# millecker/hadoop-1.0.3-gpu

Hardware: AMD Instinct MI355X
Metric: K-Means job makespan + map-tasks/sec (whole node) at 1/2/4/8 MI355X (higher is better)
Workload: dtype fp32

## Files before the change

hbmr/models/kmeans.py:

```python
from __future__ import annotations

import base64
import logging
import math
import os
import threading
import time

import numpy as np
import torch

from ..gpu.splitjob import SplitJob, SplitSpec
from ..mapred import counters as C

log = logging.getLogger("hbmr.kmeans")

K_KEY = "hbmr.kmeans.k"
D_KEY = "hbmr.kmeans.dims"
INPUT_KEY = "hbmr.kmeans.input"
SPLIT_PTS_KEY = "hbmr.split.points"
CIN_KEY = "hbmr.kmeans.centroids.in"
COUT_KEY = "hbmr.kmeans.centroids.out"
INIT_KEY = "hbmr.kmeans.centroids.init"
NCENTERS_KEY = "hbmr.kmeans.synthetic.centers"
RETURN_KEY = "hbmr.kmeans.return.centroids"
CDIR_KEY = "hbmr.kmeans.centroids.dir"
EXACT_KEY = "hbmr.kmeans.exact"
EXACT_MFMA_KEY = "hbmr.kmeans.exact.mfma"
COMBINER_KEY = "hbmr.kmeans.combiner"
BOUNDS_KEY = "hbmr.kmeans.exact.bounds"

_M32 = 0xFFFFFFFF


def _mix32(x: torch.Tensor) -> torch.Tensor:
    x = x & _M32
    x = ((x ^ (x >> 16)) * 0x45D9F3B) & _M32
    x = ((x ^ (x >> 16)) * 0x45D9F3B) & _M32
    return x ^ (x >> 16)


def _uniform(c: torch.Tensor) -> torch.Tensor:
    return (_mix32(c).to(torch.float64) + 0.5) * (1.0 / 4294967296.0)


def _gauss(c1: torch.Tensor, c2: torch.Tensor) -> torch.Tensor:
    u1 = _uniform(c1)
    u2 = _uniform(c2)
    return torch.sqrt(-2.0 * torch.log(u1)) * torch.cos(2.0 * math.pi * u2)


def synthetic_points(seed: int, start: int, n: int, d: int, centers: int, device,
                     chunk: int = 1 << 18) -> torch.Tensor:
# ... 236 lines not shown
            t = _EXACT_SKIPPED[key] = torch.zeros(1, dtype=torch.int64, device=device)
        return t


class KMeansSplitJob(SplitJob):
    collective_reduce = True
    needs_reduce = True

    def configure(self, conf):
        self.conf = conf
        self.k = conf.get_int(K_KEY, 64)
        self.d = conf.get_int(D_KEY, 128)
        self.input = conf.get(INPUT_KEY, "synthetic:100000:1")
        self.split_points = conf.get_int(SPLIT_PTS_KEY, 500_000)
        self.cin = conf.get(CIN_KEY)
        self.cout = conf.get(COUT_KEY)
        self.centers = conf.get_int(NCENTERS_KEY, self.k)
        self.fx_shift = conf.get_int("hbmr.kmeans.fx.shift", 24)
        self.cdir = conf.get(CDIR_KEY)
        self.exact = conf.get_boolean(EXACT_KEY, False)
        self.exact_dtype = torch.bfloat16 if (conf.get(EXACT_MFMA_KEY) or "f16").lower() in (
            "bf16", "bfloat16") else torch.float16
        self.bounds = conf.get_boolean(BOUNDS_KEY, True)
        self.combiner = (conf.get(COMBINER_KEY) or "delta").lower()
        if self.combiner not in ("delta", "sorted"):
            raise ValueError(f"{COMBINER_KEY} must be delta or sorted, not {self.combiner!r}")
        init = conf.get(INIT_KEY)
        if init and self.cin and STORE.host_centroids(self.cin) is None:
            STORE.put_host(self.cin, decode_centroids(init))
        if self.cin and self.cdir and STORE.host_centroids(self.cin) is None:
            path = _centroid_file(self.cdir, self.cin)
            if os.path.exists(path):
                STORE.put_host(self.cin, torch.from_numpy(np.load(path)))

    _split_memo: dict = {}

    def get_splits(self, conf, trackers):
        if self.input.startswith("synthetic:"):
            mk = (self.input, self.split_points, self.d, self.centers, tuple(trackers),
                  self.exact)
            got = KMeansSplitJob._split_memo.get(mk)
            if got is not None:
                return got
            if len(KMeansSplitJob._split_memo) > 16:
                KMeansSplitJob._split_memo.clear()
            out = KMeansSplitJob._split_memo[mk] = self._synthetic_splits(trackers)
# ... 215 lines not shown
        B = len(datas)
        sums = torch.empty(B, self.k, img.dp, dtype=torch.int64, device=ctx.device)
        counts = torch.empty(B, self.k, dtype=torch.int64, device=ctx.device)
        order = have + new + plain
        pos = {i: j for j, i in enumerate(order)}
        H = len(have)
        installed = []
        grown = None
        if have:
            ns = [datas[i].shape[0] for i in have]
            total = sum(ns)
            lab = scratch.get("labcat")
            if lab is None or lab.numel() < total:
                lab = scratch["labcat"] = torch.empty(total, dtype=torch.int32, device=ctx.device)
            need = km.delta_workspace_bytes(total, H, self.k)
            if scratch.get("dws") is None or scratch["dws"].numel() < need:
                scratch["dws"] = torch.empty(need, dtype=torch.uint8, device=ctx.device)
            hb = [bases[i] for i in have]
            bounded = self.bounds and self.combiner == "delta" and km.bounds_supported(img)
            if bounded:
                nogap = [b for b in hb if b.gap is None]
                km.assign_exact_batch([datas[i] for i in have], img, stats, lab, scratch,
                                      stream=ctx.stream, bounds=hb,
                                      skipped=_exact_skipped(self.cin, ctx.device))
                grown = {id(b): b.gap.numel() * b.gap.element_size() for b in nogap}
            else:
                km.assign_exact_batch([datas[i] for i in have], img, stats, lab, scratch,
                                      stream=ctx.stream)
            km.delta_combine([datas[i].x32 for i in have], lab, self.k, sums[:H], counts[:H],
                             scratch["dws"], hb, fx_shift=img.fx_shift, stream=ctx.stream,
                             keep_bounds=bounded)
            for i, b in zip(have, hb):
                b.S0, b.N0 = sums[pos[i]], counts[pos[i]]
                installed.append((keys[i], b))
        for i in new + plain:
            d = datas[i]
            s, c = sums[pos[i]], counts[pos[i]]
            s.zero_()
            c.zero_()
            lab = km.assign_exact(d, img, stats, scratch, stream=ctx.stream)
            need = km.workspace_bytes(d.shape[0], img.k)
            if scratch.get("ws") is None or scratch["ws"].numel() < need:
                scratch["ws"] = torch.empty(max(need, 1 << 20), dtype=torch.uint8,
                                            device=ctx.device)
            km.accumulate(d.x32, lab, img.k, s, c, fx_shift=img.fx_shift, stream=ctx.stream,
                          workspace=scratch["ws"])
            if keys[i] is not None and i in new:
# ... 386 lines not shown
```

hbmr/ops/_lib.py:

```python
from __future__ import annotations

import ctypes
import os
import threading
from pathlib import Path

import torch

_LIB_PATH = Path(__file__).resolve().parent.parent / "lib" / "libhbmr.so"
_lock = threading.Lock()
_lib = None

c_void_p = ctypes.c_void_p
c_long = ctypes.c_long
c_int = ctypes.c_int
c_uint = ctypes.c_uint
c_uint64 = ctypes.c_uint64
c_double_p = ctypes.POINTER(ctypes.c_double)

_SIGS = {
    "hbmr_kmeans_assign_bf16": (c_int, [c_void_p, c_long, c_int, c_void_p, c_void_p, c_int,
                                        c_void_p, c_void_p, c_void_p]),
    "hbmr_kmeans_accum_bf16": (c_int, [c_void_p, c_long, c_int, c_void_p, c_int, c_void_p,
                                       c_void_p, c_int, c_void_p, c_long, c_int, c_void_p]),
# ... 27 lines not shown
    "hbmr_kmeans_get_exact_kernel": (c_int, []),
    "hbmr_kmeans_refine_f32": (c_int, [c_void_p, c_long, c_int, c_int, c_void_p, c_void_p,
                                       c_void_p, c_void_p, c_int, c_int, c_void_p, c_void_p,
                                       c_void_p, c_void_p, c_void_p, c_void_p, c_int, c_void_p,
                                       c_void_p, c_void_p, c_void_p, c_void_p, c_int,
                                       c_void_p]),
    "hbmr_kmeans_refine_batch_bytes": (c_long, [c_int, c_void_p]),
    "hbmr_kmeans_assign_top3_grouped": (c_int, [c_int, c_void_p, c_void_p, c_int, c_int,
                                                c_void_p, c_void_p, c_int, c_void_p, c_void_p,
                                                c_void_p, c_void_p, c_void_p]),
    "hbmr_kmeans_refine_batch_q1g": (c_int, [c_int, c_void_p, c_int, c_int, c_int, c_void_p,
                                             c_void_p, c_void_p, c_void_p, c_void_p, c_void_p,
                                             c_void_p, c_void_p, c_void_p, c_void_p, c_void_p,
                                             c_void_p, c_long, c_void_p, c_void_p]),
    "hbmr_kmeans_refine_batch_q1": (c_int, [c_int, c_void_p, c_int, c_int, c_int, c_int,
                                            c_void_p, c_void_p, c_void_p, c_void_p, c_void_p,
                                            c_void_p, c_void_p, c_void_p, c_void_p, c_void_p,
                                            c_void_p, c_void_p, c_void_p, c_long, c_int,
                                            c_void_p, c_void_p]),
    "hbmr_kmeans_refine_batch_finish": (c_int, [c_int, c_void_p, c_void_p, c_void_p, c_int,
                                                c_int, c_void_p, c_int, c_int, c_void_p,
                                                c_void_p, c_void_p, c_void_p, c_int, c_void_p,
                                                c_int, c_void_p, c_long, c_void_p]),
    "hbmr_kmeans_accum_workspace_bytes": (c_long, [c_long, c_int]),
    "hbmr_kmeans_batch_workspace_bytes": (c_long, [c_long, c_int, c_int]),
    "hbmr_kmeans_map_batch": (c_int, [c_int, c_void_p, c_void_p, c_int, c_void_p, c_void_p, c_int,
                                      c_int, c_void_p, c_void_p, c_long, c_void_p, c_void_p,
                                      c_int, c_int, c_void_p]),
    "hbmr_kmeans_delta_workspace_bytes": (c_long, [c_long, c_int, c_int]),
    "hbmr_kmeans_delta_combine": (c_int, [c_int, c_void_p, c_void_p, c_int, c_int, c_int,
                                          c_void_p, c_void_p, c_long, c_void_p, c_void_p, c_int,
                                          c_void_p, c_void_p, c_void_p, c_void_p]),
    "hbmr_kmeans_map_batch_delta": (c_int, [c_int, c_void_p, c_void_p, c_int, c_void_p, c_void_p,
                                            c_int, c_int, c_void_p, c_void_p, c_long, c_void_p,
                                            c_void_p, c_int, c_void_p, c_void_p, c_void_p,
                                            c_void_p]),
    "hbmr_kmeans_update": (c_int, [c_void_p, c_void_p, c_int, c_int, c_int, c_int, c_int,
                                   c_void_p, c_void_p, c_void_p, c_void_p, c_void_p]),
    "hbmr_kmeans_padded_k": (c_int, [c_int]),
    "hbmr_kmeans_map_cpu_f32": (c_int, [c_void_p, c_long, c_int, c_void_p, c_int, c_void_p,
                                        c_void_p, c_void_p, c_double_p, c_int, c_int]),
    "hbmr_kmeans_map_cpu_f32_ex": (c_int, [c_void_p, c_long, c_int, c_void_p, c_int, c_void_p,
                                           c_void_p, c_void_p, c_double_p, c_int, c_int, c_int,
                                           c_void_p]),
    "hbmr_kmeans_padded_dim": (c_int, [c_int]),
    "hbmr_f32_to_bf16_pad": (c_int, [c_void_p, c_long, c_int, c_int, c_void_p, c_void_p]),
# ... 148 lines not shown
```

hbmr/ops/kmeans.py:

```python
from __future__ import annotations

import ctypes
import os
import threading

import torch

from . import _lib
from ..utils.trace import TRACE

SUPPORTED_DP = (64, 128, 256)


def _nullctx():
    import contextlib
    return contextlib.nullcontext()
FX_SHIFT = 24
NBR_L = 256


def padded_dim(d: int) -> int:
    for dp in SUPPORTED_DP:
        if d <= dp:
            return dp
# ... 302 lines not shown
        self.splits, self.img, self.stats, self.stream = splits, img, stats, stream
        self.dt = splits[0].xb.dtype
        self.ns, self.ws = _refine_ws([sp.shape[0] for sp in splits], splits[0].x32.device,
                                      scratch)
        with torch.cuda.stream(stream) if stream is not None else _nullctx():
            self.norms = img.norms(self.dt)
            self.nbr = img.neighbors()
            self.pd = img.pair_dist()
        self.labels = [None] * len(splits)
        self.lib = _lib.load()
        self.st = _lib.stream_handle(stream)

    def q1(self, i, labels_ptr, cand, scores, margin):
        sp, img = self.splits[i], self.img
        cn, cmax, ce, cemax = self.norms
        self.labels[i] = labels_ptr
        rc = self.lib.hbmr_kmeans_refine_batch_q1(
            len(self.splits), self.ns, i, img.d, img.k, img.k_pad, _ptr(sp.xnorm),
            _ptr(sp.xbn2), _ptr(sp.xerr), _ptr(cn), _ptr(cmax), _ptr(ce), _ptr(cemax),
            labels_ptr, _ptr(cand), _ptr(scores), _ptr(margin), _ptr(self.stats),
            _ptr(self.ws), self.ws.numel(), int(i == 0), _ptr(self.pd), self.st)
        _lib.check(rc, "hbmr_kmeans_refine_batch_q1")

    def finish(self):
        B = len(self.splits)
        img = self.img
        _, cmax, _, cemax = self.norms
        ni, nd, L = self.nbr
        xs = (ctypes.c_void_p * B)(*[sp.x32.data_ptr() for sp in self.splits])
        ls = (ctypes.c_void_p * B)(*[(lp.value if isinstance(lp, ctypes.c_void_p) else lp)
                                     for lp in self.labels])
        rc = self.lib.hbmr_kmeans_refine_batch_finish(
            B, self.ns, xs, ls, img.d, self.splits[0].x32.shape[1], _ptr(img.cen), img.k,
            img.k_pad, _ptr(cmax), _ptr(cemax), _ptr(ni), _ptr(nd), L, _ptr(self.stats),
            self.stats.numel(), _ptr(self.ws), self.ws.numel(), self.st)
        _lib.check(rc, "hbmr_kmeans_refine_batch_finish")


def refine_f32(split: ExactSplit, img: CentroidImage, labels, cand, scores, margin,
               stats: torch.Tensor, stream=None, scratch: dict | None = None) -> None:
    n = split.shape[0]
    if stats.dtype != torch.int64 or stats.numel() < 3:
        raise ValueError("stats must be int64 [3]")
    if labels.numel() != n or cand.numel() != 2 * n or margin.numel() != 2 * n:
        raise ValueError("labels [n], cand/margin [2n] from assign_top3 expected")
    if REFINE_VERSION >= 3:
        rb = _RefineBatch([split], img, stats, scratch, stream)
        rb.q1(0, labels.data_ptr(), cand, scores, margin)
        rb.finish()
        return
    with torch.cuda.stream(stream) if stream is not None else _nullctx():
        cn, cmax, ce, cemax = img.norms(split.xb.dtype)
        ni, nd, L = img.neighbors()
    rc = _lib.load().hbmr_kmeans_refine_f32(
        _ptr(split.x32), n, img.d, split.x32.shape[1], _ptr(split.xnorm), _ptr(split.xbn2),
        _ptr(split.xerr), _ptr(img.cen), img.k, img.k_pad, _ptr(cn), _ptr(cmax), _ptr(ce),
        _ptr(cemax), _ptr(ni), _ptr(nd), L,
        _ptr(labels), _ptr(cand), _ptr(scores), _ptr(margin), _ptr(stats), stats.numel(),
        _lib.stream_handle(stream))
# ... 6 lines not shown
    n = split.shape[0]
    dev = split.xb.device
    scratch = {} if scratch is None else scratch
    key = ("exact", n)
    bufs = scratch.get(key)
    if bufs is None:
        bufs = scratch[key] = (torch.empty(n, dtype=torch.int32, device=dev),
                               torch.empty(2 * n, dtype=torch.int32, device=dev),
                               torch.empty(n, dtype=torch.float32, device=dev),
                               torch.empty(2 * n, dtype=torch.float32, device=dev))
    lab, cand, sc, mg = bufs
    assign_top3(split.xb, img, lab, cand, sc, mg, stream=stream)
    refine_f32(split, img, lab, cand, sc, mg, stats, stream=stream, scratch=scratch)
    return lab


def bounds_supported(img: CentroidImage) -> bool:
    return REFINE_VERSION >= 3 and img.dp <= 128 and GROUPED_EXACT and FUSED_Q1 and \
        img.cen.is_cuda and _lib.load().hbmr_kmeans_get_exact_kernel() == 3


def assign_exact_batch(splits: list, img: CentroidImage, stats: torch.Tensor, out: torch.Tensor,
                       scratch: dict | None = None, stream=None, bounds: list | None = None,
                       skipped: torch.Tensor | None = None) -> None:
    if not splits:
        return
    _check_refine_dim(img)
    if bounds is not None and (len(bounds) != len(splits) or not bounds_supported(img)):
        raise ValueError("bounds: one baseline per split, grouped fused v3 assign (dp <= 128)")
    dev = splits[0].xb.device
    total = sum(sp.shape[0] for sp in splits)
    if out.dtype != torch.int32 or out.numel() < total or not out.is_contiguous():
        raise ValueError("out must be contiguous int32 with room for every split's labels")
    if stats.dtype != torch.int64 or stats.numel() < 3:
        raise ValueError("stats must be int64 [3]")
    dt = splits[0].xb.dtype
    for sp in splits:
        if sp.xb.dtype != dt or dt not in (torch.bfloat16, torch.float16) or \
                sp.xb.shape[1] != img.dp or not sp.xb.is_contiguous() or \
                not sp.x32.is_contiguous():
            raise ValueError("exact splits must hold contiguous [n, dp] rows of one 16-bit type")
    nmax = max(sp.shape[0] for sp in splits)
    scratch = {} if scratch is None else scratch
    key = ("exact-batch", nmax)
    bufs = scratch.get(key)
    if bufs is None:
        for kk in [kk for kk in scratch if isinstance(kk, tuple) and kk[0] == "exact-batch"]:
# ... 3 lines not shown
                               torch.empty(2 * nmax, dtype=torch.float32, device=dev))
    cand, sc, mg = bufs
    grouped = REFINE_VERSION >= 3 and img.dp <= 128 and GROUPED_EXACT
    with torch.cuda.stream(stream) if stream is not None else _nullctx():
        c16, ch, cn, cmax, ce, cemax = img.image16(dt)
        ni, nd, L = (None, None, 0) if grouped else img.neighbors()
        newref = None
        if bounds is not None:
            img.cen.record_stream(torch.cuda.current_stream())
            newref = img.cen.clone()
    lib = _lib.load()
    top3 = lib.hbmr_kmeans_assign_top3_f16 if dt == torch.float16 else \
        lib.hbmr_kmeans_assign_top3_bf16
    st = _lib.stream_handle(stream)
    pc, ps, pm, pst = _ptr(cand), _ptr(sc), _ptr(mg), _ptr(stats)
    pcn, pcmax, pce, pcemax, pni, pnd = (_ptr(t) for t in (cn, cmax, ce, cemax, ni, nd))
    base, off = out.data_ptr(), 0
    for g0 in range(0, len(splits), MAX_REFINE_BATCH):
        group = splits[g0:g0 + MAX_REFINE_BATCH]
        if grouped:
            off += _exact_group(group, img, stats, base + 4 * off, c16, ch, (cn, cmax, ce, cemax),
                                dt, scratch, stream, lib, st,
                                None if bounds is None else bounds[g0:g0 + MAX_REFINE_BATCH],
                                skipped, newref)
            continue
        rb = _RefineBatch(group, img, stats, scratch, stream) if REFINE_VERSION >= 3 else None
        for i, sp in enumerate(group):
            n = sp.shape[0]
            pl = ctypes.c_void_p(base + 4 * off)
            rc = top3(_ptr(sp.xb), n, img.dp, _ptr(c16), _ptr(ch), img.k_pad, pl, pc, ps, pm, st)
            _lib.check(rc, "hbmr_kmeans_assign_top3")
            if rb is not None:
                rb.q1(i, pl, cand, sc, mg)
            else:
                rc = lib.hbmr_kmeans_refine_f32(
                    _ptr(sp.x32), n, img.d, sp.x32.shape[1], _ptr(sp.xnorm), _ptr(sp.xbn2),
                    _ptr(sp.xerr), _ptr(img.cen), img.k, img.k_pad, pcn, pcmax, pce, pcemax,
                    pni, pnd, L, pl, pc, ps, pm, pst, stats.numel(), st)
                _lib.check(rc, "hbmr_kmeans_refine_f32")
            off += n
        if rb is not None:
            rb.finish()


PAIR_DIST_MAX_K = int(os.environ.get("HBMR_PAIR_DIST_MAX_K", "8192"))
NBR_NATIVE_MAX_K = int(os.environ.get("HBMR_NBR_NATIVE_MAX_K", "8192"))
GROUPED_EXACT = os.environ.get("HBMR_EXACT_GROUPED", "1") != "0"
# ... 32 lines not shown
        bws = scratch.get("bound_ws")
        if bws is None or bws.numel() < need:
            bws = scratch["bound_ws"] = torch.empty(need, dtype=torch.uint8, device=dev)
    P = ctypes.c_void_p * B
    cn, cmax, ce, cemax = norms
    refs = [b.ref for b in bases]
    for b in bases:
        b.ref = b.pending = None
    rc = lib.hbmr_kmeans_assign_top3_q1_bounded(
        B, P(*[sp.xb.data_ptr() for sp in group]), (ctypes.c_long * B)(*ns), img.dp,
        int(dt == torch.float16), _ptr(img.image16_tiled(dt)), _ptr(ch), img.k_pad, labels_ptr,
        P(*[sp.xnorm.data_ptr() for sp in group]), P(*[sp.xbn2.data_ptr() for sp in group]),
        P(*[sp.xerr.data_ptr() for sp in group]), img.d, img.k, _ptr(cn), _ptr(cmax), _ptr(ce),
        _ptr(cemax), _ptr(rb.ws), rb.ws.numel(), _ptr(rb.pd),
        P(*[b.g.data_ptr() for b in bases]), P(*[b.gap.data_ptr() for b in bases]),
        P(*[None if r is None else r.data_ptr() for r in refs]), _ptr(img.cen),
        _ptr(bws), bws.numel(), _ptr(skipped), st)
    _lib.check(rc, "hbmr_kmeans_assign_top3_q1_bounded")
    for b in bases:
        b.pending = newref


def _exact_group(group, img, stats, labels_ptr, c16, ch, norms, dt, scratch, stream, lib, st,
                 bases=None, skipped=None, newref=None):
    B = len(group)
    ns = [sp.shape[0] for sp in group]
    N = sum(ns)
    dev = group[0].xb.device
    P = ctypes.c_void_p * B
    xs = P(*[sp.xb.data_ptr() for sp in group])
    nsa = (ctypes.c_long * B)(*ns)
    if bases is not None:
        rb = _RefineBatch(group, img, stats, scratch, stream)
        if TRACE.on:
            TRACE.instant("kmeans.top3_launch", n=B)
        _bounded_group(group, bases, img, labels_ptr, ch, norms, dt, scratch, stream, lib, st, rb,
                       skipped, newref)
        o = 0
        for i in range(B):
            rb.labels[i] = labels_ptr + 4 * o
            o += ns[i]
        rb.finish()
        return N
    if FUSED_Q1 and img.dp <= 128:
        rb = _RefineBatch(group, img, stats, scratch, stream)
        if TRACE.on:
            TRACE.instant("kmeans.top3_launch", n=B)
        cn, cmax, ce, cemax = norms
        rc = lib.hbmr_kmeans_assign_top3_q1_grouped(
            B, xs, nsa, img.dp, int(dt == torch.float16), _ptr(c16),
            _ptr(img.image16_tiled(dt)), _ptr(ch), img.k_pad,
            labels_ptr, P(*[sp.xnorm.data_ptr() for sp in group]),
            P(*[sp.xbn2.data_ptr() for sp in group]), P(*[sp.xerr.data_ptr() for sp in group]),
            img.d, img.k, _ptr(cn), _ptr(cmax), _ptr(ce), _ptr(cemax), _ptr(rb.ws),
            rb.ws.numel(), _ptr(rb.pd), st)
        _lib.check(rc, "hbmr_kmeans_assign_top3_q1_grouped")
        o = 0
        for i in range(B):
            rb.labels[i] = labels_ptr + 4 * o
            o += ns[i]
        rb.finish()
        return N
    key = ("exact-group", N)
    bufs = scratch.get(key)
    if bufs is None:
# ... 199 lines not shown
```

native/include/hbmr/hbmr.h:

```cpp
#pragma once
#include <stddef.h>
#include <stdint.h>

#ifdef __cplusplus
extern "C" {
#endif

typedef struct ihipStream_t* hbmr_stream_t;

#ifndef HBMR_NO_HIP_DECLS
#include <hip/hip_runtime_api.h>
int hbmr_kmeans_assign_bf16(const void* X, long n, int dp, const void* C, const float* chalf,
                            int k_pad, int32_t* labels, float* scores, hipStream_t st);
int hbmr_kmeans_accum_bf16(const void* X, long n, int dp, const int32_t* labels, int k,
                           long long* sums, long long* counts, int fx_shift, void* ws,
                           long ws_bytes, int mode, hipStream_t st);
int hbmr_kmeans_accum_f32(const float* X, long n, int dp, const int32_t* labels, int k,
                          long long* sums, long long* counts, int fx_shift, void* ws,
                          long ws_bytes, int mode, hipStream_t st);
int hbmr_kmeans_assign_top3_bf16(const void* X, long n, int dp, const void* C, const float* chalf,
                                 int k_pad, int32_t* labels, int32_t* cand, float* scores,
                                 float* margin, hipStream_t st);
int hbmr_kmeans_assign_top3_f16(const void* X, long n, int dp, const void* C, const float* chalf,
                                int k_pad, int32_t* labels, int32_t* cand, float* scores,
// ... 37 lines not shown
                                    int f16, const void* C, const float* chalf, int k_pad,
                                    int32_t* labels, int32_t* cand, float* scores, float* margin,
                                    hipStream_t st);
int hbmr_kmeans_refine_batch_q1g(int nsplit, const long* ns, int d, int k, int k_pad,
                                 const float* const* xnorm, const float* const* xbn2,
                                 const float* const* xerr, const float* cnorm, const float* cmax,
                                 const float* cerr, const float* cerrmax, const int32_t* labels,
                                 const int32_t* cand, const float* scores, const float* margin,
                                 void* ws, long ws_bytes, const float* dcc, hipStream_t st);
long hbmr_kmeans_refine_batch_bytes(int nsplit, const long* ns);
int hbmr_kmeans_refine_batch_q1(int nsplit, const long* ns, int s, int d, int k, int k_pad,
                                const float* xnorm, const float* xbn2, const float* xerr,
                                const float* cnorm, const float* cmax, const float* cerr,
                                const float* cerrmax, const int32_t* labels, const int32_t* cand,
                                const float* scores, const float* margin,
                                unsigned long long* stats, void* ws, long ws_bytes, int reset,
                                const float* dcc, hipStream_t st);
int hbmr_kmeans_refine_batch_finish(int nsplit, const long* ns, const float* const* x32,
                                    int32_t* const* labels, int d, int ldx, const float* C32,
                                    int k, int k_pad, const float* cmax, const float* cerrmax,
                                    const int32_t* nbr_idx, const float* nbr_dist, int L,
                                    unsigned long long* stats, int nstats, void* ws,
                                    long ws_bytes, hipStream_t st);
int hbmr_kmeans_update(const long long* sums, const long long* counts, int fx_shift, int k, int d,
                       int dp, int k_pad, float* cen, void* cbf, float* chalf, float* shift2,
                       hipStream_t st);
int hbmr_kmeans_map_batch(int ntasks, const void* const* X, const long* n, int dp,
                          const void* C, const float* chalf, int k_pad, int k, int32_t* labels,
                          void* ws, long ws_bytes, long long* sums, long long* counts,
                          int fx_shift, int zero_outputs, hipStream_t st);
int hbmr_f32_to_bf16_pad(const float* src, long n, int d, int dp, void* dst, hipStream_t st);
#endif
int hbmr_kmeans_padded_dim(int d);

#ifndef HBMR_NO_HIP_DECLS
int hbmr_radix_sort_pairs_u64(uint64_t* keys, uint32_t* vals, uint64_t* tkeys, uint32_t* tvals,
                              long n, int begin_bit, int end_bit, void* ws, long ws_bytes,
                              hipStream_t st);
int hbmr_teragen(long first_row, long nrows, void* out, hipStream_t st);
int hbmr_tera_keys(const void* records, long n, int stride, uint64_t* hi, uint64_t* lo,
                   hipStream_t st);
int hbmr_gather_u64(const uint64_t* src, const uint32_t* perm, long n, uint64_t* dst,
                    hipStream_t st);
int hbmr_gather_records(const void* src, const uint32_t* perm, long n, int record_bytes, void* dst,
                        hipStream_t st);
int hbmr_split_offsets(const uint64_t* hi, const uint64_t* lo, long n, const uint64_t* shi,
// ... 132 lines not shown
```

native/kernels/kmeans.hip:

```cpp
#include "common.h"
#include "../include/hbmr/hbmr.h"
#include <algorithm>
#include <cstdlib>
#include <cstring>
#include <type_traits>

namespace {

constexpr int kWaves = 4;
constexpr int kThreads = kWaves * HBMR_WAVE;
constexpr int kCK = 64;

template <bool F16>
__device__ __forceinline__ f32x16 mfma32x32x16(bf16x8 a, bf16x8 b, f32x16 c) {
  if constexpr (F16)
    return __builtin_amdgcn_mfma_f32_32x32x16_f16(__builtin_bit_cast(f16x8, a),
                                                  __builtin_bit_cast(f16x8, b), c, 0, 0, 0);
  else
    return __builtin_amdgcn_mfma_f32_32x32x16_bf16(a, b, c, 0, 0, 0);
}

template <int D> struct AssignCfg {
  static constexpr int KS = D / 16;
  static constexpr int CPR = D / 8;
// ... 2610 lines not shown
      const int b = 128 * m + 32 * h + 4 * sub;
      const bool ok = b < d;
      const float4 a = *reinterpret_cast<const float4*>(r + (ok ? b : 0));
      float* o = v + 16 * m + 4 * h;
      o[0] = ok ? a.x : 0.f; o[1] = ok ? a.y : 0.f; o[2] = ok ? a.z : 0.f; o[3] = ok ? a.w : 0.f;
    }
  }
}

__device__ __forceinline__ float row_sum8f(float v) {
  v += __shfl_xor(v, 1);
  v += __shfl_xor(v, 2);
  v += __shfl_xor(v, 4);
  return v;
}

__device__ __forceinline__ double row_sum8(double v) {
  v += dpp_f64<0xB1>(v);
  v += dpp_f64<0x4E>(v);
  v += dpp_f64<0x141>(v);
  return v;
}

template <int NM>
__global__ __launch_bounds__(256) void kmeans_refine_q2_kernel(
    const RefineTable tbl, int d, int ldx, const float* __restrict__ C32, int k,
    const float* __restrict__ cmax, const float* __restrict__ cerrmax, double pack_rel,
    const uint32_t* __restrict__ qcount, const ExactQ1* __restrict__ q1, long cap1,
    uint32_t* __restrict__ q2count, ExactQ2* __restrict__ q2, long cap2,
    unsigned long long* __restrict__ sstats) {
  constexpr uint32_t kPerBlk = 4 * kQ2Per;
  constexpr uint32_t kBuf = 256;
  const int tid = threadIdx.x, lane = tid & 63, wave = tid >> 6;
  const int grp = lane / kQ2Lanes, sub = lane % kQ2Lanes;
  __shared__ ExactQ2 sbuf[kBuf];
  __shared__ uint32_t sn, sbase;
  __shared__ unsigned long long cnt[2];
  if (tid < 2) cnt[tid] = 0;
  if (tid == 0) sn = 0;
  __syncthreads();
  const double inflate = 1.0 + 0x1p-20;
  const double gam = (double)(d + 2) * 0x1p-23 * 1.01;
  const double cem = (double)cerrmax[0] * inflate;
  const double cm = (double)cmax[0] * inflate + cem;
  uint32_t c1[kQShards];
  uint32_t total = 0;
#pragma unroll
  for (int j = 0; j < kQShards; ++j) {
    c1[j] = qcount[j];
// ... 32 lines not shown
    float f0 = 0.f, f1 = 0.f, f2 = 0.f;
#pragma unroll
    for (int i = 0; i < 16 * NM; ++i) {
      const float e0 = xf[i] - c0[i], e1 = xf[i] - c1r[i], e2 = xf[i] - c2[i];
      f0 = fmaf(e0, e0, f0);
      f1 = fmaf(e1, e1, f1);
      f2 = fmaf(e2, e2, f2);
    }
    f0 = row_sum8f(f0);
    f1 = row_sum8f(f1);
    f2 = row_sum8f(f2);
    const double rel = (double)(16 * NM + 8) * 0x1p-24 * 1.01, aeps = 0x1p-120;
    int w = q.b;
    double dw = f0;
    if ((double)f1 < dw || ((double)f1 == dw && q.s < w)) { w = q.s; dw = f1; }
    if (t_real && ((double)f2 < dw || ((double)f2 == dw && q.t < w))) { w = q.t; dw = f2; }
    const double whi = dw * (1.0 + rel) + aeps;
    auto beats = [&](double dj) { return dj * (1.0 - rel) - aeps > whi; };
    bool separated = isfinite(whi) &&
                     (w == q.b || beats(f0)) && (w == q.s || beats(f1)) &&
                     (!t_real || w == q.t || beats(f2));
    dw = whi;
    bool certified = !t_real && separated;
    if (t_real && separated) {
      const double xn = ((double)q.xn + (double)q.xe) * inflate;
      const double x2 = (double)q.x2;
      const double amax = ((double)q.xe + cem) * inflate;
      const double st = (double)q.sb - (double)q.m3;
      double et, dl_t;
      exact_bound(st, cm, xn, x2, amax, gam, pack_rel, et, dl_t);
      certified = 0.5 * (x2 - dw) - x2 * 0x1p-23 > st + et && dl_t >= 2.0 * amax;
    }
    if (have && sub == 0 && certified && w != q.b) {
      tbl.labels[q.split][q.row] = w;
      atomicAdd(&cnt[0], 1ull);
    }
    const bool spill = have && sub == 0 && !certified;
    const unsigned long long m = __ballot(spill);
    if (m) {
      uint32_t b2 = 0;
      if (lane == 0) b2 = atomicAdd(&sn, (uint32_t)__popcll(m));
      b2 = __shfl(b2, 0);
      if (spill) {
        ExactQ2 o;
        o.row = q.row;
        o.split = q.split;
        o.w = w;
        o.pad = 0;
        o.dw = dw;
        sbuf[b2 + lane_rank(m)] = o;
      }
    }
    __syncthreads();
    if (sn > kBuf - kPerBlk) flush();
  }
  __syncthreads();
  if (sn) flush();
  if (tid < 2 && cnt[tid]) atomicAdd(sstats + 4 * shard + 1 + tid, cnt[tid]);
}

template <int NM>
__global__ __launch_bounds__(256) void kmeans_refine_q3_kernel(
    const RefineTable tbl, int d, int ldx, const float* __restrict__ C32, int k,
    const int32_t* __restrict__ nbr_idx, const float* __restrict__ nbr_dist, int L,
    const uint32_t* __restrict__ q2count, const ExactQ2* __restrict__ q2, long cap2,
    unsigned long long* __restrict__ sstats, int nstats) {
  const int tid = threadIdx.x, lane = tid & 63;
  const int grp = lane / kRefineGroup, sub = lane % kRefineGroup;
  __shared__ unsigned long long cnt[3];
  if (tid < 3) cnt[tid] = 0;
  __syncthreads();
  uint32_t c2[kQShards];
  uint32_t total = 0;
#pragma unroll
  for (int j = 0; j < kQShards; ++j) {
    c2[j] = q2count[j];
    total += c2[j];
  }
  const uint32_t nwaves = gridDim.x * 4;
  const uint32_t gw = blockIdx.x * 4 + (tid >> 6);
  for (uint32_t base = gw * 4; base < total; base += nwaves * 4) {
    const uint32_t idx = base + grp;
    const bool have = idx < total;
    const ExactQ2 q = q2[shard_slot(c2, cap2, have ? idx : base)];
    int32_t* lab = tbl.labels[q.split];
    const int b0 = lab[q.row];
    double xv[8 * NM];
    {
      float xf[8 * NM];
      load_row8<NM>(tbl.x32[q.split] + (size_t)q.row * ldx, d, sub, xf);
#pragma unroll
      for (int i = 0; i < 8 * NM; ++i) xv[i] = (double)xf[i];
    }
    const int w0 = q.w;
    int w = w0;
    double dw;
    {
      const float* c0p[1] = {C32 + (size_t)w0 * d};
      double d0[1];
      rows_dist2<NM, 1>(xv, c0p, d, sub, d0);
      dw = d0[0];
    }
    const double r0 = sqrt(dw);
    bool done = false;
    const int32_t* ni = nbr_idx + (size_t)w0 * L;
    const float* nd = nbr_dist + (size_t)w0 * L;
    const float* cw0 = C32 + (size_t)w0 * d;
    int evals = 0;
    for (int jj = 0; jj < L; jj += kElkanStep) {
      const double lim = (r0 + sqrt(dw)) * (1.0 + 0x1p-40);
      if ((double)nd[jj] > lim) {
        done = true;
        break;
      }
      int jv[kElkanStep];
      const float* cp[kElkanStep];
#pragma unroll
      for (int v = 0; v < kElkanStep; ++v) {
        const bool ok = jj + v < L && (double)nd[jj + v] <= lim;
        jv[v] = ok ? ni[jj + v] : -1;
        cp[v] = ok ? C32 + (size_t)jv[v] * d : cw0;
      }
      double dj[kElkanStep];
      rows_dist2<NM, kElkanStep>(xv, cp, d, sub, dj);
      evals += kElkanStep;
#pragma unroll
      for (int v = 0; v < kElkanStep; ++v)
        if (jv[v] >= 0 && (dj[v] < dw || (dj[v] == dw && jv[v] < w))) { w = jv[v]; dw = dj[v]; }
    }
    const bool full = !done && L < k;
    if (full) {
      for (int j = 0; j < k; j += 4) {
        const float* cp[4];
#pragma unroll
        for (int v = 0; v < 4; ++v) cp[v] = C32 + (size_t)(j + v < k ? j + v : j) * d;
        double dj[4];
        rows_dist2<NM, 4>(xv, cp, d, sub, dj);
#pragma unroll
        for (int v = 0; v < 4; ++v)
          if (j + v < k && (dj[v] < dw || (dj[v] == dw && j + v < w))) { w = j + v; dw = dj[v]; }
      }
    }
    if (have && sub == 0) {
      atomicAdd(&cnt[1], (unsigned long long)evals);
      if (full) atomicAdd(&cnt[2], 1ull);
      if (w != b0) atomicAdd(&cnt[0], 1ull);
      lab[q.row] = w;
    }
  }
  __syncthreads();
  const int sh = blockIdx.x % (kQShards / 2);
  if (tid == 0 && cnt[0]) atomicAdd(sstats + 4 * sh + 1, cnt[0]);
  if (tid == 1 && cnt[1]) atomicAdd(sstats + 4 * sh + 3, cnt[1]);
  if (tid == 2 && cnt[2]) atomicAdd(sstats + 4 * (sh + kQShards / 2) + 3, cnt[2]);
}

__global__ void kmeans_refine_stats_kernel(const unsigned long long* __restrict__ ss,
                                           unsigned long long* __restrict__ stats, int nstats) {
  const int t = threadIdx.x;
  if (t >= 5 || (t >= 3 && nstats < 5)) return;
  unsigned long long v = 0;
  if (t < 3) {
    for (int j = 0; j < kQShards; ++j) v += ss[4 * j + t];
  } else {
    for (int j = 0; j < kQShards / 2; ++j) v += ss[4 * (j + (t - 3) * (kQShards / 2)) + 3];
  }
  if (v) stats[t] += v;
}

template <int D, bool F16>
// ... 908 lines not shown
    t.xbn2[i] = xbn2[i];
    t.xerr[i] = xerr[i];
    total += ns[i];
    nb += ceil_div(ns[i], 256 * kQ1Per);
  }
  t.blk[nsplit] = nb;
  t.total = total;
  const RefineLayout Ly = refine_layout(nsplit, ns);
  if (ws_bytes < (long)Ly.bytes) return (int)hipErrorInvalidValue;
  char* w = static_cast<char*>(ws);
  uint32_t* c1 = reinterpret_cast<uint32_t*>(w);
  HBMR_RETURN_IF_ERROR(hipMemsetAsync(c1, 0, kHdrClear, st));
  if (nb == 0) return 0;
  int tb = 0;
  while ((1 << tb) < k_pad / 32) ++tb;
  const double pack_rel = ldexp(1.0, 4 + tb - 23);
  hipLaunchKernelGGL(kmeans_refine_q1_grouped_kernel, dim3((unsigned)nb), dim3(256), 0, st, t, d,
                     k, cnorm, cmax, cerr, cerrmax, pack_rel, labels, cand, scores, margin, c1,
                     reinterpret_cast<ExactQ1*>(w + Ly.off1), Ly.cap1,
                     reinterpret_cast<unsigned long long*>(w + kStatsOff), dcc);
  return (int)hipGetLastError();
}

int hbmr_kmeans_refine_batch_finish(int nsplit, const long* ns, const float* const* x32,
                                    int32_t* const* labels, int d, int ldx, const float* C32,
                                    int k, int k_pad, const float* cmax, const float* cerrmax,
                                    const int32_t* nbr_idx, const float* nbr_dist, int L,
                                    unsigned long long* stats, int nstats, void* ws,
                                    long ws_bytes, hipStream_t st) {
  if (nsplit <= 0 || nsplit > kMaxGroup || d > ldx || d > kRefineMaxDp || d % 8 || ldx % 4 ||
      k <= 0 || k_pad < k || L < 1 || L > k || nstats < 3 || ((uintptr_t)C32 & 15) ||
      ((uintptr_t)ws & 255))
    return (int)hipErrorInvalidValue;
  const RefineLayout Ly = refine_layout(nsplit, ns);
  if (ws_bytes < (long)Ly.bytes) return (int)hipErrorInvalidValue;
  RefineTable tbl;
  std::memset(&tbl, 0, sizeof(tbl));
  tbl.nsplit = nsplit;
  for (int i = 0; i < nsplit; ++i) {
    if ((uintptr_t)x32[i] & 15) return (int)hipErrorInvalidValue;
    tbl.x32[i] = x32[i];
    tbl.labels[i] = labels[i];
  }
  int tb = 0;
  while ((1 << tb) < k_pad / 32) ++tb;
  const double pack_rel = ldexp(1.0, 4 + tb - 23);
  char* w = static_cast<char*>(ws);
  uint32_t* c1 = reinterpret_cast<uint32_t*>(w);
  uint32_t* c2 = c1 + kQShards;
  const ExactQ1* q1 = reinterpret_cast<const ExactQ1*>(w + Ly.off1);
  ExactQ2* q2 = reinterpret_cast<ExactQ2*>(w + Ly.off2);
  unsigned long long* ss = reinterpret_cast<unsigned long long*>(w + kStatsOff);
  const unsigned g3 = std::max(1u, Ly.g2);
  if (d <= 128) {
    hipLaunchKernelGGL(kmeans_refine_q2_kernel<1>, dim3(Ly.g2), dim3(256), 0, st, tbl, d, ldx,
                       C32, k, cmax, cerrmax, pack_rel, c1, q1, Ly.cap1, c2, q2, Ly.cap2, ss);
    HBMR_RETURN_IF_ERROR(hipGetLastError());
    hipLaunchKernelGGL(kmeans_refine_q3_kernel<1>, dim3(g3), dim3(256), 0, st, tbl, d, ldx, C32,
                       k, nbr_idx, nbr_dist, L, c2, q2, Ly.cap2, ss, nstats);
  } else {
    hipLaunchKernelGGL(kmeans_refine_q2_kernel<2>, dim3(Ly.g2), dim3(256), 0, st, tbl, d, ldx,
                       C32, k, cmax, cerrmax, pack_rel, c1, q1, Ly.cap1, c2, q2, Ly.cap2, ss);
    HBMR_RETURN_IF_ERROR(hipGetLastError());
    hipLaunchKernelGGL(kmeans_refine_q3_kernel<2>, dim3(g3), dim3(256), 0, st, tbl, d, ldx, C32,
                       k, nbr_idx, nbr_dist, L, c2, q2, Ly.cap2, ss, nstats);
  }
  HBMR_RETURN_IF_ERROR(hipGetLastError());
  hipLaunchKernelGGL(kmeans_refine_stats_kernel, dim3(1), dim3(64), 0, st, ss, stats, nstats);
  return (int)hipGetLastError();
}

}
```

Before: 9936.

## Write certified Elkan-style gap bounds from refine q2/q3 kernels for bounded reassignment

The exact refine q2 and q3 kernels now compute a conservative lower bound on the gap between each point's winning centroid distance and the second-best distance, and write it into per-split gap tensors. The bounded delta path uses these gaps by default (new refined config key, default on). Tighter gaps should let later iterations skip more points whose assignment cannot change. The cost is extra double-precision arithmetic and stores inside the refine kernels, and added tracking of second-best distances in q3. GapTable is used in the kernels but its definition is not shown.

```diff
diff --git a/hbmr/models/kmeans.py b/hbmr/models/kmeans.py
--- a/hbmr/models/kmeans.py
+++ b/hbmr/models/kmeans.py
@@ -29,6 +29,7 @@
 EXACT_MFMA_KEY = "hbmr.kmeans.exact.mfma"
 COMBINER_KEY = "hbmr.kmeans.combiner"
 BOUNDS_KEY = "hbmr.kmeans.exact.bounds"
+BOUNDS_REFINED_KEY = "hbmr.kmeans.exact.bounds.refined"
 
 _M32 = 0xFFFFFFFF
 
@@ -311,6 +312,7 @@
         self.exact_dtype = torch.bfloat16 if (conf.get(EXACT_MFMA_KEY) or "f16").lower() in (
             "bf16", "bfloat16") else torch.float16
         self.bounds = conf.get_boolean(BOUNDS_KEY, True)
+        self.bounds_refined = conf.get_boolean(BOUNDS_REFINED_KEY, True)
         self.combiner = (conf.get(COMBINER_KEY) or "delta").lower()
         if self.combiner not in ("delta", "sorted"):
             raise ValueError(f"{COMBINER_KEY} must be delta or sorted, not {self.combiner!r}")
@@ -572,7 +574,8 @@
                 nogap = [b for b in hb if b.gap is None]
                 km.assign_exact_batch([datas[i] for i in have], img, stats, lab, scratch,
                                       stream=ctx.stream, bounds=hb,
-                                      skipped=_exact_skipped(self.cin, ctx.device))
+                                      skipped=_exact_skipped(self.cin, ctx.device),
+                                      refined=self.bounds_refined)
                 grown = {id(b): b.gap.numel() * b.gap.element_size() for b in nogap}
             else:
                 km.assign_exact_batch([datas[i] for i in have], img, stats, lab, scratch,
diff --git a/hbmr/ops/_lib.py b/hbmr/ops/_lib.py
--- a/hbmr/ops/_lib.py
+++ b/hbmr/ops/_lib.py
@@ -73,6 +73,11 @@
                                                 c_int, c_void_p, c_int, c_int, c_void_p,
                                                 c_void_p, c_void_p, c_void_p, c_int, c_void_p,
                                                 c_int, c_void_p, c_long, c_void_p]),
+    "hbmr_kmeans_refine_batch_finish_gaps": (c_int, [c_int, c_void_p, c_void_p, c_void_p, c_int,
+                                                     c_int, c_void_p, c_int, c_int, c_void_p,
+                                                     c_void_p, c_void_p, c_void_p, c_int,
+                                                     c_void_p, c_int, c_void_p, c_long, c_void_p,
+                                                     c_void_p]),
     "hbmr_kmeans_accum_workspace_bytes": (c_long, [c_long, c_int]),
     "hbmr_kmeans_batch_workspace_bytes": (c_long, [c_long, c_int, c_int]),
     "hbmr_kmeans_map_batch": (c_int, [c_int, c_void_p, c_void_p, c_int, c_void_p, c_void_p, c_int,
diff --git a/hbmr/ops/kmeans.py b/hbmr/ops/kmeans.py
--- a/hbmr/ops/kmeans.py
+++ b/hbmr/ops/kmeans.py
@@ -348,7 +348,7 @@
             _ptr(self.ws), self.ws.numel(), int(i == 0), _ptr(self.pd), self.st)
         _lib.check(rc, "hbmr_kmeans_refine_batch_q1")
 
-    def finish(self):
+    def finish(self, gaps: list | None = None):
         B = len(self.splits)
         img = self.img
         _, cmax, _, cemax = self.norms
@@ -356,11 +356,21 @@
         xs = (ctypes.c_void_p * B)(*[sp.x32.data_ptr() for sp in self.splits])
         ls = (ctypes.c_void_p * B)(*[(lp.value if isinstance(lp, ctypes.c_void_p) else lp)
                                      for lp in self.labels])
-        rc = self.lib.hbmr_kmeans_refine_batch_finish(
-            B, self.ns, xs, ls, img.d, self.splits[0].x32.shape[1], _ptr(img.cen), img.k,
-            img.k_pad, _ptr(cmax), _ptr(cemax), _ptr(ni), _ptr(nd), L, _ptr(self.stats),
-            self.stats.numel(), _ptr(self.ws), self.ws.numel(), self.st)
-        _lib.check(rc, "hbmr_kmeans_refine_batch_finish")
+        args = (B, self.ns, xs, ls, img.d, self.splits[0].x32.shape[1], _ptr(img.cen), img.k,
+                img.k_pad, _ptr(cmax), _ptr(cemax), _ptr(ni), _ptr(nd), L, _ptr(self.stats),
+                self.stats.numel(), _ptr(self.ws), self.ws.numel(), self.st)
+        if gaps is None:
+            rc = self.lib.hbmr_kmeans_refine_batch_finish(*args)
+            _lib.check(rc, "hbmr_kmeans_refine_batch_finish")
+            return
+        if len(gaps) != B or any(g is not None and (g.dtype != torch.float32 or
+                                                    g.numel() != sp.shape[0] or
+                                                    not g.is_contiguous())
+                                 for g, sp in zip(gaps, self.splits)):
+            raise ValueError("gaps: one contiguous fp32 [n] tensor (or None) per split")
+        gs = (ctypes.c_void_p * B)(*[None if g is None else g.data_ptr() for g in gaps])
+        rc = self.lib.hbmr_kmeans_refine_batch_finish_gaps(*args, gs)
+        _lib.check(rc, "hbmr_kmeans_refine_batch_finish_gaps")
 
 
 def refine_f32(split: ExactSplit, img: CentroidImage, labels, cand, scores, margin,
@@ -413,7 +423,7 @@
 
 def assign_exact_batch(splits: list, img: CentroidImage, stats: torch.Tensor, out: torch.Tensor,
                        scratch: dict | None = None, stream=None, bounds: list | None = None,
-                       skipped: torch.Tensor | None = None) -> None:
+                       skipped: torch.Tensor | None = None, refined: bool = False) -> None:
     if not splits:
         return
     _check_refine_dim(img)
@@ -463,7 +473,7 @@
             off += _exact_group(group, img, stats, base + 4 * off, c16, ch, (cn, cmax, ce, cemax),
                                 dt, scratch, stream, lib, st,
                                 None if bounds is None else bounds[g0:g0 + MAX_REFINE_BATCH],
-                                skipped, newref)
+                                skipped, newref, refined)
             continue
         rb = _RefineBatch(group, img, stats, scratch, stream) if REFINE_VERSION >= 3 else None
         for i, sp in enumerate(group):
@@ -542,7 +552,7 @@
 
 
 def _exact_group(group, img, stats, labels_ptr, c16, ch, norms, dt, scratch, stream, lib, st,
-                 bases=None, skipped=None, newref=None):
+                 bases=None, skipped=None, newref=None, refined=False):
     B = len(group)
     ns = [sp.shape[0] for sp in group]
     N = sum(ns)
@@ -560,7 +570,7 @@
         for i in range(B):
             rb.labels[i] = labels_ptr + 4 * o
             o += ns[i]
-        rb.finish()
+        rb.finish([b.gap for b in bases] if refined else None)
         return N
     if FUSED_Q1 and img.dp <= 128:
         rb = _RefineBatch(group, img, stats, scratch, stream)
diff --git a/native/include/hbmr/hbmr.h b/native/include/hbmr/hbmr.h
--- a/native/include/hbmr/hbmr.h
+++ b/native/include/hbmr/hbmr.h
@@ -83,6 +83,13 @@
                                     const int32_t* nbr_idx, const float* nbr_dist, int L,
                                     unsigned long long* stats, int nstats, void* ws,
                                     long ws_bytes, hipStream_t st);
+int hbmr_kmeans_refine_batch_finish_gaps(int nsplit, const long* ns, const float* const* x32,
+                                         int32_t* const* labels, int d, int ldx,
+                                         const float* C32, int k, int k_pad, const float* cmax,
+                                         const float* cerrmax, const int32_t* nbr_idx,
+                                         const float* nbr_dist, int L, unsigned long long* stats,
+                                         int nstats, void* ws, long ws_bytes, hipStream_t st,
+                                         float* const* gap);
 int hbmr_kmeans_update(const long long* sums, const long long* counts, int fx_shift, int k, int d,
                        int dp, int k_pad, float* cen, void* cbf, float* chalf, float* shift2,
                        hipStream_t st);
diff --git a/native/kernels/kmeans.hip b/native/kernels/kmeans.hip
--- a/native/kernels/kmeans.hip
+++ b/native/kernels/kmeans.hip
@@ -2656,9 +2656,30 @@
   return v;
 }
 
+__device__ __forceinline__ float q2_gap(const ExactQ1& q, int w, bool t_real, float f0, float f1,
+                                        float f2, double rel, double aeps, double whi,
+                                        double ceil_t) {
+  auto below = [&](double fj) {
+    return fj * (1.0 - rel) - aeps - whi - (fj + whi) * 0x1p-50;
+  };
+  double delta = __builtin_inf();
+  if (q.b != w) delta = fmin(delta, below(f0));
+  if (q.s != w) delta = fmin(delta, below(f1));
+  if (t_real) {
+    if (q.t != w) delta = fmin(delta, below(f2));
+    const double x2 = (double)q.x2;
+    delta = fmin(delta, 2.0 * ((0.5 * (x2 - whi) - x2 * 0x1p-23) - ceil_t));
+  }
+  if (!(delta > 0.0) || !isfinite(delta)) return 0.f;
+  delta *= 1.0 - 0x1p-30;
+  const double r = sqrt(whi) * (1.0 + 0x1p-40);
+  const double g = delta / (sqrt(whi + delta) * (1.0 + 0x1p-40) + r) * (1.0 - 0x1p-30);
+  return isfinite(g) ? fmaxf(0.f, __double2float_rd(g)) : 0.f;
+}
+
 template <int NM>
 __global__ __launch_bounds__(256) void kmeans_refine_q2_kernel(
-    const RefineTable tbl, int d, int ldx, const float* __restrict__ C32, int k,
+    const RefineTable tbl, const GapTable gt, int d, int ldx, const float* __restrict__ C32, int k,
     const float* __restrict__ cmax, const float* __restrict__ cerrmax, double pack_rel,
     const uint32_t* __restrict__ qcount, const ExactQ1* __restrict__ q1, long cap1,
     uint32_t* __restrict__ q2count, ExactQ2* __restrict__ q2, long cap2,
@@ -2737,6 +2758,7 @@
                      (!t_real || w == q.t || beats(f2));
     dw = whi;
     bool certified = !t_real && separated;
+    double ceil_t = 0.0;
     if (t_real && separated) {
       const double xn = ((double)q.xn + (double)q.xe) * inflate;
       const double x2 = (double)q.x2;
@@ -2744,11 +2766,16 @@
       const double st = (double)q.sb - (double)q.m3;
       double et, dl_t;
       exact_bound(st, cm, xn, x2, amax, gam, pack_rel, et, dl_t);
-      certified = 0.5 * (x2 - dw) - x2 * 0x1p-23 > st + et && dl_t >= 2.0 * amax;
-    }
-    if (have && sub == 0 && certified && w != q.b) {
-      tbl.labels[q.split][q.row] = w;
-      atomicAdd(&cnt[0], 1ull);
+      ceil_t = st + et;
+      certified = 0.5 * (x2 - dw) - x2 * 0x1p-23 > ceil_t && dl_t >= 2.0 * amax;
+    }
+    if (have && sub == 0 && certified) {
+      if (w != q.b) {
+        tbl.labels[q.split][q.row] = w;
+        atomicAdd(&cnt[0], 1ull);
+      }
+      float* gp = gt.gap[q.split];
+      if (gp != nullptr) gp[q.row] = q2_gap(q, w, t_real, f0, f1, f2, rel, aeps, whi, ceil_t);
     }
     const bool spill = have && sub == 0 && !certified;
     const unsigned long long m = __ballot(spill);
@@ -2774,9 +2801,18 @@
   if (tid < 2 && cnt[tid]) atomicAdd(sstats + 4 * shard + 1 + tid, cnt[tid]);
 }
 
+__device__ __forceinline__ float q3_gap(double dw, double d2, float ndlo, double r0, double rel) {
+  const double rw = sqrt(dw) * (1.0 + rel);
+  const double lo = fmin(sqrt(d2) * (1.0 - rel), (double)ndlo - r0 * (1.0 + rel));
+  double g = lo - rw - (rw + r0) * 0x1p-40;
+  if (!(g > 0.0) || !isfinite(g)) return 0.f;
+  g *= (1.0 - 0x1p-30) * (1.0 - 0x1p-30);
+  return fmaxf(0.f, __double2float_rd(g));
+}
+
 template <int NM>
 __global__ __launch_bounds__(256) void kmeans_refine_q3_kernel(
-    const RefineTable tbl, int d, int ldx, const float* __restrict__ C32, int k,
+    const RefineTable tbl, const GapTable gt, int d, int ldx, const float* __restrict__ C32, int k,
     const int32_t* __restrict__ nbr_idx, const float* __restrict__ nbr_dist, int L,
     const uint32_t* __restrict__ q2count, const ExactQ2* __restrict__ q2, long cap2,
     unsigned long long* __restrict__ sstats, int nstats) {
@@ -2822,9 +2858,12 @@
     const float* nd = nbr_dist + (size_t)w0 * L;
     const float* cw0 = C32 + (size_t)w0 * d;
     int evals = 0;
+    double d2 = __builtin_inf();
+    float ndlo = __builtin_inff();
     for (int jj = 0; jj < L; jj += kElkanStep) {
       const double lim = (r0 + sqrt(dw)) * (1.0 + 0x1p-40);
       if ((double)nd[jj] > lim) {
+        ndlo = fminf(ndlo, nd[jj]);
         done = true;
         break;
       }
@@ -2833,6 +2872,7 @@
 #pragma unroll
       for (int v = 0; v < kElkanStep; ++v) {
         const bool ok = jj + v < L && (double)nd[jj + v] <= lim;
+        if (!ok && jj + v < L) ndlo = fminf(ndlo, nd[jj + v]);
         jv[v] = ok ? ni[jj + v] : -1;
         cp[v] = ok ? C32 + (size_t)jv[v] * d : cw0;
       }
@@ -2841,10 +2881,20 @@
       evals += kElkanStep;
 #pragma unroll
       for (int v = 0; v < kElkanStep; ++v)
-        if (jv[v] >= 0 && (dj[v] < dw || (dj[v] == dw && jv[v] < w))) { w = jv[v]; dw = dj[v]; }
+        if (jv[v] >= 0) {
+          if (dj[v] < dw || (dj[v] == dw && jv[v] < w)) {
+            d2 = dw;
+            w = jv[v];
+            dw = dj[v];
+          } else if (jv[v] != w) {
+            d2 = fmin(d2, dj[v]);
+          }
+        }
     }
     const bool full = !done && L < k;
     if (full) {
+      d2 = __builtin_inf();
+      ndlo = __builtin_inff();
       for (int j = 0; j < k; j += 4) {
         const float* cp[4];
 #pragma unroll
@@ -2853,7 +2903,15 @@
         rows_dist2<NM, 4>(xv, cp, d, sub, dj);
 #pragma unroll
         for (int v = 0; v < 4; ++v)
-          if (j + v < k && (dj[v] < dw || (dj[v] == dw && j + v < w))) { w = j + v; dw = dj[v]; }
+          if (j + v < k) {
+            if (dj[v] < dw || (dj[v] == dw && j + v < w)) {
+              d2 = dw;
+              w = j + v;
+              dw = dj[v];
+            } else if (j + v != w) {
+              d2 = fmin(d2, dj[v]);
+            }
+          }
       }
     }
     if (have && sub == 0) {
@@ -2861,6 +2919,9 @@
       if (full) atomicAdd(&cnt[2], 1ull);
       if (w != b0) atomicAdd(&cnt[0], 1ull);
       lab[q.row] = w;
+      float* gp = gt.gap[q.split];
+      if (gp != nullptr)
+        gp[q.row] = q3_gap(dw, d2, ndlo, r0, (double)(d + 4) * 0x1p-53 * 1.01);
     }
   }
   __syncthreads();
@@ -3815,12 +3876,13 @@
   return (int)hipGetLastError();
 }
 
-int hbmr_kmeans_refine_batch_finish(int nsplit, const long* ns, const float* const* x32,
-                                    int32_t* const* labels, int d, int ldx, const float* C32,
-                                    int k, int k_pad, const float* cmax, const float* cerrmax,
-                                    const int32_t* nbr_idx, const float* nbr_dist, int L,
-                                    unsigned long long* stats, int nstats, void* ws,
-                                    long ws_bytes, hipStream_t st) {
+int hbmr_kmeans_refine_batch_finish_gaps(int nsplit, const long* ns, const float* const* x32,
+                                         int32_t* const* labels, int d, int ldx,
+                                         const float* C32, int k, int k_pad, const float* cmax,
+                                         const float* cerrmax, const int32_t* nbr_idx,
+                                         const float* nbr_dist, int L, unsigned long long* stats,
+                                         int nstats, void* ws, long ws_bytes, hipStream_t st,
+                                         float* const* gap) {
   if (nsplit <= 0 || nsplit > kMaxGroup || d > ldx || d > kRefineMaxDp || d % 8 || ldx % 4 ||
       k <= 0 || k_pad < k || L < 1 || L > k || nstats < 3 || ((uintptr_t)C32 & 15) ||
       ((uintptr_t)ws & 255))
@@ -3835,6 +3897,10 @@
     tbl.x32[i] = x32[i];
     tbl.labels[i] = labels[i];
   }
+  GapTable gt;
+  std::memset(&gt, 0, sizeof(gt));
+  if (gap != nullptr)
+    for (int i = 0; i < nsplit; ++i) gt.gap[i] = gap[i];
   int tb = 0;
   while ((1 << tb) < k_pad / 32) ++tb;
   const double pack_rel = ldexp(1.0, 4 + tb - 23);
@@ -3846,21 +3912,32 @@
   unsigned long long* ss = reinterpret_cast<unsigned long long*>(w + kStatsOff);
   const unsigned g3 = std::max(1u, Ly.g2);
   if (d <= 128) {
-    hipLaunchKernelGGL(kmeans_refine_q2_kernel<1>, dim3(Ly.g2), dim3(256), 0, st, tbl, d, ldx,
-                       C32, k, cmax, cerrmax, pack_rel, c1, q1, Ly.cap1, c2, q2, Ly.cap2, ss);
+    hipLaunchKernelGGL(kmeans_refine_q2_kernel<1>, dim3(Ly.g2), dim3(256), 0, st, tbl, gt, d,
+                       ldx, C32, k, cmax, cerrmax, pack_rel, c1, q1, Ly.cap1, c2, q2, Ly.cap2, ss);
     HBMR_RETURN_IF_ERROR(hipGetLastError());
-    hipLaunchKernelGGL(kmeans_refine_q3_kernel<1>, dim3(g3), dim3(256), 0, st, tbl, d, ldx, C32,
-                       k, nbr_idx, nbr_dist, L, c2, q2, Ly.cap2, ss, nstats);
+    hipLaunchKernelGGL(kmeans_refine_q3_kernel<1>, dim3(g3), dim3(256), 0, st, tbl, gt, d, ldx,
+                       C32, k, nbr_idx, nbr_dist, L, c2, q2, Ly.cap2, ss, nstats);
   } else {
-    hipLaunchKernelGGL(kmeans_refine_q2_kernel<2>, dim3(Ly.g2), dim3(256), 0, st, tbl, d, ldx,
-                       C32, k, cmax, cerrmax, pack_rel, c1, q1, Ly.cap1, c2, q2, Ly.cap2, ss);
+    hipLaunchKernelGGL(kmeans_refine_q2_kernel<2>, dim3(Ly.g2), dim3(256), 0, st, tbl, gt, d,
+                       ldx, C32, k, cmax, cerrmax, pack_rel, c1, q1, Ly.cap1, c2, q2, Ly.cap2, ss);
     HBMR_RETURN_IF_ERROR(hipGetLastError());
-    hipLaunchKernelGGL(kmeans_refine_q3_kernel<2>, dim3(g3), dim3(256), 0, st, tbl, d, ldx, C32,
-                       k, nbr_idx, nbr_dist, L, c2, q2, Ly.cap2, ss, nstats);
+    hipLaunchKernelGGL(kmeans_refine_q3_kernel<2>, dim3(g3), dim3(256), 0, st, tbl, gt, d, ldx,
+                       C32, k, nbr_idx, nbr_dist, L, c2, q2, Ly.cap2, ss, nstats);
   }
   HBMR_RETURN_IF_ERROR(hipGetLastError());
   hipLaunchKernelGGL(kmeans_refine_stats_kernel, dim3(1), dim3(64), 0, st, ss, stats, nstats);
   return (int)hipGetLastError();
 }
 
-}
+int hbmr_kmeans_refine_batch_finish(int nsplit, const long* ns, const float* const* x32,
+                                    int32_t* const* labels, int d, int ldx, const float* C32,
+                                    int k, int k_pad, const float* cmax, const float* cerrmax,
+                                    const int32_t* nbr_idx, const float* nbr_dist, int L,
+                                    unsigned long long* stats, int nstats, void* ws,
+                                    long ws_bytes, hipStream_t st) {
+  return hbmr_kmeans_refine_batch_finish_gaps(nsplit, ns, x32, labels, d, ldx, C32, k, k_pad, cmax,
+                                              cerrmax, nbr_idx, nbr_dist, L, stats, nstats, ws,
+                                              ws_bytes, st, nullptr);
+}
+
+}
```

Measured after the change: 9444. -5.0%, worse.
